# fudan-zvg/S-NeRF

Hardware: AMD Instinct MI355X
Metric: rays/sec (train step) (higher is better)
Workload: dtype bf16; 1 GPU; S-NeRF path A (MipNerfModel) train step, nuScenes-like 1600x900 rays, 64 proposal + 128 fine evals/ray (192 spp), hidden 1024, rgb_layer 3, cone + contraction + IPE-96

## Files before the change

include/snerf_hip.h:

```cpp
#ifndef SNERF_HIP_H
#define SNERF_HIP_H
#ifdef __cplusplus
extern "C" {
#endif

#define SNERF_DT_F32 0
#define SNERF_DT_BF16 1
#define SNERF_DT_F16 2
#define SNERF_DT_F64 3
#define SNERF_DT_BF16X3 4
#define SNERF_ACT_NONE 0
#define SNERF_ACT_RELU 1
#define SNERF_ACT_MASK 2
#define SNERF_ACT_RELU_BITS 3
#define SNERF_ACT_MASK_BITS 4

int snerf_version(void);
int snerf_last_hip_error(void);
int snerf_debug_lds_scribble(int seed, void* stream);

int snerf_linear_fwd(const void* A, long lda, const void* W, long ldw, const float* bias, void* Y, long ldy,
                     const void* aux, long ldaux, float* colsum, float* colsum_ws, int M, int N, int K, int n_store,
                     int act, int dtype, int out_f32, int variant, void* stream);

// ... 241 lines not shown
                             void* const* bits, void* const* dz, const long* dz_ld, float* const* g_bias, float* ws, long ws_floats, long M,
                             int dtype, void* stream);
int snerf_fcolour_fwd(const void* CB, long ldCB, const void* wstream, long n_frags, const float* bias, int n_blocks, float* raw_rgb,
                      void* const* acts, const long* act_ld, void* const* bits, long M, int variant, void* stream);
long snerf_fcolour_bwd_ws_floats(long M);
int snerf_fcolour_bwd(const float* d_raw_rgb, const void* wstream, long n_frags, void* const* bits, void* const* dC, const long* dC_ld,
                      void* dB, long dB_ld, float* const* g_bias, float* ws, long ws_floats, long M, void* stream);
int snerf_fcolour_fwd_dt(const void* CB, long ldCB, const void* wstream, long n_frags, const float* bias, int n_blocks, float* raw_rgb,
                         void* const* acts, const long* act_ld, void* const* bits, long M, int variant, int dtype, void* stream);
int snerf_fcolour_bwd_dt(const float* d_raw_rgb, const void* wstream, long n_frags, void* const* bits, void* const* dC, const long* dC_ld,
                         void* dB, long dB_ld, float* const* g_bias, float* ws, long ws_floats, long M, int dtype, void* stream);

long snerf_fchain_bwd_ws_floats(int net, long M);
int snerf_fchain_bwd(int net, const float* d_raw, const void* wstream, long n_frags, void* const* bits, void* const* dz, const long* dz_ld,
                     float* const* g_bias, float* ws, long ws_floats, long M, void* stream);
int snerf_fchain_bwd_dt(int net, const float* d_raw, const void* wstream, long n_frags, void* const* bits, void* const* dz, const long* dz_ld,
                        float* const* g_bias, float* ws, long ws_floats, long M, int dtype, void* stream);

long snerf_linear_wgrad_ws_floats(int M, int N, int K, long ldz, long ldx, int dtype, int variant);
int snerf_linear_wgrad_det(const void* Z, long ldz, const void* X, long ldx, float* dW, long ldw, const void* zeros, int M, int N, int K,
                           int n_valid, int k_valid, int dtype, int variant, float* ws, long ws_floats, void* stream);
int snerf_colsum_f32_det(const float* x, long ld, long M, int C, float* out, void* stream);

int snerf_classic_get_rays(int H, int W, double focal, double cx, double cy, const float* c2w_host, float* rays_o, float* rays_d, void* stream);
int snerf_classic_ndc_rays(int H, int W, double focal, float near, const float* rays_o, const float* rays_d, long n, float* o_out,
                           float* d_out, void* stream);
int snerf_classic_ray_batch(int H, int W, double focal, double cx, double cy, const float* c2w_host, const float* c2w_static_host,
                            const float* rays_o, const float* rays_d, long n, int ndc, float near, float far, const float* depths,
                            int use_viewdirs, float* rows, int ld, void* stream);

int snerf_zip_encode_bwd_binned(int pass, const float* tdist, const float* origins, const float* directions, const float* radii,
                                const float* base_x, const float* base_y, const float* deg_jitter, const int* offsets,
                                const int* grid_sizes, const void* grad_feat, long ld, float* grad_table, long R, int S, int L, int C, int n,
                                int m, float Sl, int H, float std_scale, int feat_dtype, const int* ksplit_host, const int* level_rows_host,
                                int* counts, void* wg_offsets, const long* starts, void* rec_row, float* rec_val, long capacity, void* g64,
                                long g64_rows, const int* scale_exp, void* stream);
int snerf_colsum_wide_f32(const float* x, long ld, long M, int C, float* out, int deterministic, void* stream);
int snerf_zip_glo_modulate(const void* X, long ldx, const float* SS, long ldss, long R, int S, int B, void* out, long ldo, int dtype, void* stream);
int snerf_zip_glo_modulate_bwd(const void* dXm, long lddxm, const void* X, long ldx, const float* SS, long ldss, const float* d_head, long ldh,
                               int n_head, long R, int S, int B, void* dX, long lddx, float* dSS, long lddss, float* dxsum, long ldsum,
                               int dtype, void* stream);
int snerf_zip_bin_scale(const void* grad_feat, long ld, long rows, int cols, int feat_dtype, int* scale_exp, void* stream);

int snerf_zip_encode_ray_bwd(const float* tdist, const float* origins, const float* directions, const float* radii, const float* base_x,
                             const float* base_y, const float* deg_jitter, const void* table, const int* offsets, const int* grid_sizes,
                             const void* grad_feat, long ld, long R, int S, int L, int C, int n, int m, float Sl, int H, float std_scale,
// ... 28 lines not shown
```

snerf_amd/csrc/elementwise.hip:

```cpp
#include "common.h"

struct AdamArgs {
  float lr, b1, b2, eps, grad_scale, grad_max_val;
  int zero_grad, nonfinite;
  const int* step_dev;
  const float* lr_dev;
  const float* clip_coef;
  int step;
  unsigned long long* dropped;
};

__device__ __forceinline__ float adam_clean_grad(float g, const AdamArgs& a, float coef) {
  g *= a.grad_scale * coef;
  if (a.grad_max_val > 0.f && g == g) g = fminf(fmaxf(g, -a.grad_max_val), a.grad_max_val);
  if (a.nonfinite == 1) g = (fabsf(g) <= 3.402823466e+38f) ? g : 0.f;
  else if (a.nonfinite == 2) g = (g != g) ? 0.f : fminf(fmaxf(g, -3.402823466e+38f), 3.402823466e+38f);
  return g;
}

__device__ __forceinline__ void adam_update(float& p, float& m, float& v, float gk, float b1, float b2, float step_size, float bc2_sqrt, float eps) {
#pragma clang fp contract(off)
  m = b1 * m + (1.f - b1) * gk;
  v = b2 * v + ((1.f - b2) * gk) * gk;
  p = p - (step_size * m) / (sqrtf(v) / bc2_sqrt + eps);
// ... 480 lines not shown
      (n_tiles > 0 && (tiles == nullptr || (((uintptr_t)tiles) & 15)))) return SNERF_ERR_ARG;
  if (n_b < 0 || (n_b > 0 && (idx_b == nullptr || dst_b == nullptr || (((uintptr_t)idx_b) & 15)))) return SNERF_ERR_ARG;
  const long want = (n + 1023) / 1024, want_b = (n_b + 1023) / 1024;
  const int gblocks = (int)(want < 4096 ? want : 4096), tblocks = (n_tiles + 3) / 4, bblocks = (int)(want_b < 1024 ? want_b : 1024);
  const dim3 g((unsigned)(gblocks + tblocks + bblocks)), b(256);
  const PackTile* tl = (const PackTile*)tiles;
  hipStream_t s = (hipStream_t)stream;
  if (dtype == SNERF_DT_F32) hipLaunchKernelGGL(gather_pack_tiles_kernel<float>, g, b, 0, s, flat, idx, n, (float*)dst, tl, n_tiles, tblocks, gblocks, idx_b, n_b, dst_b);
  else if (dtype == SNERF_DT_BF16) hipLaunchKernelGGL(gather_pack_tiles_kernel<__bf16>, g, b, 0, s, flat, idx, n, (__bf16*)dst, tl, n_tiles, tblocks, gblocks, idx_b, n_b, dst_b);
  else if (dtype == SNERF_DT_F16) hipLaunchKernelGGL(gather_pack_tiles_kernel<_Float16>, g, b, 0, s, flat, idx, n, (_Float16*)dst, tl, n_tiles, tblocks, gblocks, idx_b, n_b, dst_b);
  else return SNERF_ERR_ARG;
  return snerf_check_launch();
}

extern "C" int snerf_gather_pack_tiles(const float* flat, const int* idx, long n, void* dst, int dtype, const int* tiles, int n_tiles, void* stream) {
  return gather_pack_launch(flat, idx, n, dst, dtype, tiles, n_tiles, nullptr, 0, nullptr, stream);
}

extern "C" int snerf_gather_pack_pair(const float* flat, const int* idx, long n, void* dst, int dtype, const int* tiles, int n_tiles, const int* idx32,
                                      long n32, float* dst32, void* stream) {
  return gather_pack_launch(flat, idx, n, dst, dtype, tiles, n_tiles, idx32, n32, dst32, stream);
}

extern "C" int snerf_version() { return 3; }
int g_snerf_last_hip_error = 0;
extern "C" int snerf_last_hip_error() { return g_snerf_last_hip_error; }

__global__ __launch_bounds__(1024) void lds_scribble_kernel(unsigned seed, unsigned* sink) {
  extern __shared__ unsigned scribble[];
  unsigned h = seed * 2654435761u + blockIdx.x * 40503u + 17u;
  for (int i = threadIdx.x; i < 160 * 1024 / 4; i += 1024) {
    h = (h ^ (unsigned)i) * 1664525u + 1013904223u;
    scribble[i] = (h >> 7) ^ (h << 13);
  }
  __syncthreads();
  if (scribble[(seed + threadIdx.x) % (160 * 1024 / 4)] == 0x5eed5eedu && sink != nullptr) sink[0] = seed;
}
extern "C" int snerf_debug_lds_scribble(int seed, void* stream) {
  static bool attr = false;
  if (!attr) { (void)hipFuncSetAttribute((const void*)lds_scribble_kernel, hipFuncAttributeMaxDynamicSharedMemorySize, 160 * 1024); attr = true; }
  hipLaunchKernelGGL(lds_scribble_kernel, dim3(4096), dim3(1024), 160 * 1024, (hipStream_t)stream, (unsigned)seed, (unsigned*)nullptr);
  return snerf_check_launch();
}

__global__ __launch_bounds__(256) void split8_cast_kernel(const float* __restrict__ src, long ld_src, long M, int C, int G, _Float16* __restrict__ dst,
                                                          long ld_dst, int weight) {
  typedef _Float16 f16x8 __attribute__((ext_vector_type(8)));
// ... 34 lines not shown
```

snerf_amd/csrc/gemm.hip:

```cpp
#include "common.h"
#include <cstdlib>
#include <type_traits>

#define ACT_NONE 0
#define ACT_RELU 1
#define ACT_MASK 2
typedef unsigned short u16x2 __attribute__((ext_vector_type(2)));
#define ACT_RELU_BITS 3
#define ACT_MASK_BITS 4

typedef unsigned u32x4 __attribute__((ext_vector_type(4)));
typedef unsigned u32x2 __attribute__((ext_vector_type(2)));

struct GemmNT {
  const void* A; long lda;
  const void* W; long ldw;
  const float* bias;
  void* Y; long ldy;
  const void* aux; long ldaux;
  float* colsum;
  int M, N, K, n_store, act, out_f32, vec_store;
  float* colsum_ws; int fast_epi;
  int det;
  int dbg;
// ... 1223 lines not shown
    if ((variant & 1) && N % 256 == 0) return launch_nt<__bf16, 256, 256, 2, 4, true>(p, s);
    return launch_nt<__bf16, 128, 128, 2, 2, true>(p, s);
  }
  if (p8) return launch_nt8p(p, s);
  if (dtype == SNERF_DT_BF16 && (variant & 12) && N % 256 == 0) return launch_nt8(p, s);
  if (dtype == SNERF_DT_F32) return launch_nt<float, 128, 128, 2, 2>(p, s);
  if ((variant & 1) && N % 256 == 0) return launch_nt<__bf16, 256, 256, 2, 4>(p, s);
  return launch_nt<__bf16, 128, 128, 2, 2>(p, s);
}

struct GemmTN {
  const void* Z; long ldz;
  const void* X; long ldx;
  float* dW; long ldw;
  const void* zeros;
  int M, N, K, n_valid, k_valid, m_chunk;
  int tiles, slices;
  int split;
  float* part;
  long part_stride;
  int part_ld;
};

template <typename T, bool TR, int TN_STAGES, bool F16 = false>
__global__ __launch_bounds__(256) void gemm_tn_kernel(GemmTN p) {
  extern __shared__ __attribute__((aligned(16))) char smem[];
  constexpr int EPC = 16 / (int)sizeof(T);
  constexpr int ROWB = 128 * (int)sizeof(T);
  constexpr int MT = sizeof(T) == 4 ? 16 : 32;
  constexpr int TILEB = MT * ROWB;
  constexpr int RPI = 1024 / ROWB;
  constexpr int LI = MT / RPI / 4;
  const int tid = threadIdx.x, lane = tid & 63;
  const int wave = __builtin_amdgcn_readfirstlane(tid >> 6);
  const int wn = wave >> 1, wk = wave & 1;
  const int tiles_k = (p.K + 127) / 128;
  const int ntile = p.tiles;
  int slice, tile;
  {
    const int b = (int)blockIdx.x, xcd = b & 7, idx = b >> 3;
    const int full = p.slices >> 3;
    const int extra = p.slices & 7;
    const int mine = full + (xcd < extra ? 1 : 0);
    if (idx >= mine * ntile) return;
    slice = (idx / ntile) * 8 + xcd;
    tile = idx % ntile;
// ... 104 lines not shown
#pragma unroll
          for (int j = 0; j < 2; ++j) mma32t<F16>(acc[i][j], a[i].v, b[j].v);
      }
    }
  }
#pragma unroll
  for (int i = 0; i < 2; ++i)
#pragma unroll
    for (int j = 0; j < 2; ++j) {
      int k = k0 + wk * 64 + j * 32 + (lane & 31);
      if (p.split == 1) k = ((k >> 7) << 6) | (k & 63);
#pragma unroll
      for (int r = 0; r < 16; ++r) {
        int n = n0 + wn * 64 + i * 32 + (r & 3) + 8 * (r >> 2) + 4 * (lane >> 5);
        if (p.split == 1) n = ((n >> 7) << 6) | (n & 63);
        if (n < p.n_valid && k < p.k_valid) {
          if (p.part != nullptr) p.part[(long)slice * p.part_stride + (long)n * p.part_ld + k] = acc[i][j][r];
          else atomicAdd(p.dW + (long)n * p.ldw + k, acc[i][j][r]);
        }
      }
    }
}

template <bool SPLIT, bool F16 = false>
__global__ __launch_bounds__(512) void gemm_tn8_kernel(GemmTN p) {
  extern __shared__ __attribute__((aligned(16))) char smem[];
  typedef __bf16 T;
  typedef __attribute__((address_space(3))) bf16x4* lds_b4;
  constexpr int HALF = 64 * 256;
  const int tid = threadIdx.x, lane = tid & 63;
  const int wave = __builtin_amdgcn_readfirstlane(tid >> 6);
  const int wr = wave >> 2, wc = wave & 3;
  const int tiles_k = (p.K + 255) >> 8, tiles_n = (p.N + 255) >> 8;
  const int ntile = tiles_k * tiles_n;
  const int id = xcd_remap((int)blockIdx.x, (int)gridDim.x);
  const int tile = id % ntile, chunk = id / ntile;
  const int n0 = (tile / tiles_k) << 8, k0 = (tile % tiles_k) << 8;
  const int mbeg = chunk * p.m_chunk;
  const int rows = min(p.M, mbeg + p.m_chunk) - mbeg;
  const int KT = (rows + 63) >> 6;
  const T* __restrict__ Z = (const T*)p.Z + (long)mbeg * p.ldz + n0;
  const bool xhi = !SPLIT && p.split == 2;
  const T* __restrict__ X = (const T*)p.X + (long)mbeg * p.ldx + (xhi ? 2 * k0 : k0);
  const int xcols = xhi ? ((p.K - 1) >> 6) * 128 + ((p.K - 1) & 63) + 1 - 2 * k0 : p.K - k0;
  const int zbytes = (rows - 1) * (int)p.ldz * 2 + (p.N - n0) * 2, xbytes = (rows - 1) * (int)p.ldx * 2 + xcols * 2;
  const int zstep = 64 * (int)p.ldz * 2, xstep = 64 * (int)p.ldx * 2;

  const int lrow = lane >> 4, lch = lane & 15;
  const int lc = (lch ^ (4 * lrow)) * 8;
  constexpr int xhalf = SPLIT ? 128 : 64;
  const int zcol = ((lc >> 6) * 128 + (lc & 63)) * 2;
  const int xcol = SPLIT ? (((lc >> 6) * 128) + ((lc >> 5) & 1) * 32 + (lc & 31)) * 2 : ((lc >> 5) * (xhi ? 128 : 64) + (lc & 31)) * 2;
  int zrel[2], xrel[2];
#pragma unroll
  for (int i = 0; i < 2; ++i) {
    const int r = (wave * 2 + i) * 4 + lrow;
    zrel[i] = r * (int)p.ldz * 2 + zcol;
    xrel[i] = r * (int)p.ldx * 2 + xcol;
  }
  int s_kt = 0;
  auto stage = [&](int db, int which) __attribute__((always_inline)) {
    char* dst = smem + (db * 4 + which) * HALF + wave * 2048;
    if (which < 2) {
      const int off = s_kt * zstep;
      const int left = zbytes - off;
      const __amdgpu_buffer_rsrc_t r = __builtin_amdgcn_make_buffer_rsrc((void*)((const char*)Z + off), 0, left > 0 ? left : 0, 0x00020000);
      __builtin_amdgcn_raw_ptr_buffer_load_lds(r, (lds_ptr_t)dst, 16, zrel[0] + which * 128, 0, 0, 0);
      __builtin_amdgcn_raw_ptr_buffer_load_lds(r, (lds_ptr_t)(dst + 1024), 16, zrel[1] + which * 128, 0, 0, 0);
    } else {
      const int off = s_kt * xstep;
      const int left = xbytes - off;
      const __amdgpu_buffer_rsrc_t r = __builtin_amdgcn_make_buffer_rsrc((void*)((const char*)X + off), 0, left > 0 ? left : 0, 0x00020000);
      __builtin_amdgcn_raw_ptr_buffer_load_lds(r, (lds_ptr_t)dst, 16, xrel[0] + (which - 2) * xhalf, 0, 0, 0);
      __builtin_amdgcn_raw_ptr_buffer_load_lds(r, (lds_ptr_t)(dst + 1024), 16, xrel[1] + (which - 2) * xhalf, 0, 0, 0);
    }
  };

  const int g4 = lane >> 4, pl = lane & 15, prow = pl >> 2;
  const int frow = (8 * (g4 >> 1) + prow) * 256;
  const int fsub = ((pl & 1) << 3);
  int zc[2], xc1;
#pragma unroll
  for (int i2 = 0; i2 < 2; ++i2) zc[i2] = ((((wr * 64 + i2 * 32 + 16 * (g4 & 1)) >> 3) + ((pl & 3) >> 1)) ^ (4 * prow)) << 4;
  xc1 = ((((wc * 32 + 16 * (g4 & 1)) >> 3) + ((pl & 3) >> 1)) ^ (4 * prow)) << 4;
  bf16x8 aF[2][4], bS[2][4];
  const unsigned lds0 = (unsigned)(size_t)smem;
  auto lds_frag = [&](unsigned addr) __attribute__((always_inline)) {
    bf16x4 lo, hi;
    asm volatile("ds_read_b64_tr_b16 %0, %2\n\tds_read_b64_tr_b16 %1, %2 offset:1024" : "=&v"(lo), "=&v"(hi) : "v"(addr));
    return __builtin_shufflevector(lo, hi, 0, 1, 2, 3, 4, 5, 6, 7);
  };
  const unsigned za[2] = {lds0 + frow + zc[0] + fsub, lds0 + frow + zc[1] + fsub};
  const unsigned xa = lds0 + frow + xc1 + fsub;
  auto lds_a = [&](int db, int h, int i2, int ks) __attribute__((always_inline)) {
// ... 17 lines not shown
  };
  auto end_phase = [&]() __attribute__((always_inline)) {
    __builtin_amdgcn_sched_barrier(0);
    __builtin_amdgcn_s_barrier();
    __builtin_amdgcn_sched_barrier(0);
  };

  stage(0, 2); stage(0, 0); stage(0, 3); stage(0, 1);
  ++s_kt;
  stage(1, 3); stage(1, 0); stage(1, 2); stage(1, 1);
  ++s_kt;
  asm volatile("s_waitcnt vmcnt(10)" ::: "memory");
  __builtin_amdgcn_s_barrier();
#pragma unroll
  for (int ks = 0; ks < 4; ++ks) {
    aF[0][ks] = lds_a(0, 0, 0, ks);
    aF[1][ks] = lds_a(0, 0, 1, ks);
    bS[0][ks] = lds_b(0, 0, ks);
  }
  __builtin_amdgcn_s_waitcnt(0xC07F);
  __builtin_amdgcn_sched_barrier(0);
  __builtin_amdgcn_s_barrier();

  auto ktile = [&](auto db_tag) __attribute__((always_inline)) {
    constexpr int db = decltype(db_tag)::value;
    constexpr int F = db, S = 1 - db;
    if (wr == 1) { stage(db, 2 + F); wait_load(); }
#pragma unroll
    for (int ks = 0; ks < 4; ++ks) {
      bS[S][ks] = lds_b(db, S, ks);
      mma32t<F16>(acc[0][F], aF[0][ks], bS[F][ks]);
      mma32t<F16>(acc[1][F], aF[1][ks], bS[F][ks]);
      __builtin_amdgcn_sched_barrier(0);
    }
    if (wr == 0) { stage(db, 2 + F); wait_load(); }
    end_phase();
    if (wr == 1) { stage(db, 0); wait_load(); }
#pragma unroll
    for (int ks = 0; ks < 4; ++ks)
#pragma unroll
      for (int i2 = 0; i2 < 2; ++i2) {
        mma32t<F16>(acc[i2][S], aF[i2][ks], bS[S][ks]);
        aF[i2][ks] = lds_a(db, 1, i2, ks);
        __builtin_amdgcn_sched_barrier(0);
      }
    if (wr == 0) { stage(db, 0); wait_load(); }
    end_phase();
    if (wr == 1) { stage(db, 2 + S); wait_load(); }
    constexpr bool skip3 = S == 1 && SPLIT, skip4 = F == 1 && SPLIT;
#pragma unroll
    for (int ks = 0; ks < 4; ++ks) {
      if constexpr (!skip3) {
        mma32t<F16>(acc[2][S], aF[0][ks], bS[S][ks]);
        mma32t<F16>(acc[3][S], aF[1][ks], bS[S][ks]);
      }
      bS[S][ks] = lds_b(db ^ 1, S, ks);
      __builtin_amdgcn_sched_barrier(0);
    }
    if (wr == 0) { stage(db, 2 + S); wait_load(); }
    end_phase();
    if (wr == 1) { stage(db, 1); ++s_kt; wait_load(); }
#pragma unroll
    for (int ks = 0; ks < 4; ++ks)
#pragma unroll
      for (int i2 = 0; i2 < 2; ++i2) {
        if constexpr (!skip4) mma32t<F16>(acc[2 + i2][F], aF[i2][ks], bS[F][ks]);
        aF[i2][ks] = lds_a(db ^ 1, 0, i2, ks);
        __builtin_amdgcn_sched_barrier(0);
      }
    if (wr == 0) { stage(db, 1); ++s_kt; wait_load(); }
    end_phase();
  };
  for (int t = 0; t < KT; t += 2) {
    ktile(std::integral_constant<int, 0>{});
    if (t + 1 < KT) ktile(std::integral_constant<int, 1>{});
  }
  asm volatile("s_waitcnt vmcnt(0)" ::: "memory");

#pragma unroll
  for (int i = 0; i < 4; ++i)
#pragma unroll
    for (int j = 0; j < 2; ++j) {
      int k = k0 + wc * 64 + j * 32 + (lane & 31);
      if constexpr (SPLIT) {
        if (i >= 2 && j == 1) continue;
        k = k0 + (wc >> 1) * 128 + j * 64 + (wc & 1) * 32 + (lane & 31);
        k = ((k >> 7) << 6) | (k & 63);
      }
#pragma unroll
      for (int r = 0; r < 16; ++r) {
        int n = n0 + wr * 128 + i * 32 + (r & 3) + 8 * (r >> 2) + 4 * (lane >> 5);
        if constexpr (SPLIT) n = ((n >> 7) << 6) | (n & 63);
        if (n < p.n_valid && k < p.k_valid) {
          if (p.part != nullptr) p.part[(long)chunk * p.part_stride + (long)n * p.part_ld + k] = acc[i][j][r];
          else atomicAdd(p.dW + (long)n * p.ldw + k, acc[i][j][r]);
        }
      }
    }
}

// ... 40 lines not shown
#pragma unroll
  for (int w = 0; w < W; ++w) sm[g][lane][w] = s[w];
  __syncthreads();
  if (g == 0 && live) {
    float* dst = dW + (long)n * ldw + k;
#pragma unroll
    for (int w = 0; w < W; ++w) {
      float t = sm[0][lane][w];
#pragma unroll
      for (int q = 1; q < G; ++q) t += sm[q][lane][w];
      dst[w] += t;
    }
  }
}

struct TnPlan {
  bool use8;
  int slices;
  int m_chunk;
  int part_ld;
  long part_stride;
};

static TnPlan tn_plan(int M, int N, int K, long ldz, long ldx, int dtype, int variant, bool fold = false) {
  static int n_cu = 0;
  if (n_cu == 0) {
    int dev = 0;
    hipDeviceProp_t prop;
    n_cu = 256;
    if (hipGetDevice(&dev) == hipSuccess && hipGetDeviceProperties(&prop, dev) == hipSuccess && prop.multiProcessorCount > 0)
      n_cu = prop.multiProcessorCount;
  }
  TnPlan pl{};
  if ((variant & 2) && dtype == SNERF_DT_BF16 && N % 256 == 0 && K >= 256 && M >= 4096 && ldz * 2 * 65 < (1L << 31) && ldx * 2 * 65 < (1L << 31)) {
    const int t8 = (N / 256) * ((K + 255) / 256);
    int ch = n_cu / t8;
    ch = ch < 1 ? 1 : ch;
    long mc = ((long)M + ch - 1) / ch;
    mc = ((mc + 127) / 128) * 128;
    const long lim = (1L << 30) / ((ldz > ldx ? ldz : ldx) * 2);
    if (mc > lim) mc = lim / 128 * 128;
    if (!(fold && M <= 131072 && mc < 512)) {
      pl.use8 = true; pl.m_chunk = (int)mc; pl.slices = (int)((M + mc - 1) / mc);
      pl.part_ld = ((K + 255) / 256) * 256; pl.part_stride = (long)N * pl.part_ld;
      return pl;
    }
  }
  const int tiles = ((N + 127) / 128) * ((K + 127) / 128);
  const int target = (variant & 64) ? 4096 : (variant & 32) ? 2048 : (variant & 16) ? 512 : 1024;
  int chunks = (target + tiles - 1) / tiles;
  int m_chunk = (M + chunks - 1) / chunks;
  m_chunk = ((m_chunk + 255) / 256) * 256;
  const int floor_rows = (fold && M <= 131072) ? 256 : 1024;
  if (m_chunk < floor_rows) m_chunk = floor_rows;
  pl.use8 = false; pl.m_chunk = m_chunk; pl.slices = (M + m_chunk - 1) / m_chunk;
// ... 83 lines not shown
      hipLaunchKernelGGL(tn_fold_kernel<false>, dim3((k_valid + 255) / 256, n_valid), dim3(256), 0, (hipStream_t)stream, ws, pl.part_stride,
                         pl.part_ld, pl.slices, n_valid, k_valid, dW, ldw);
  }
  return snerf_check_launch();
}

extern "C" int snerf_linear_wgrad(const void* Z, long ldz, const void* X, long ldx, float* dW, long ldw, const void* zeros,
                                  int M, int N, int K, int n_valid, int k_valid, int dtype, int variant, void* stream) {
  return wgrad_launch(Z, ldz, X, ldx, dW, ldw, zeros, M, N, K, n_valid, k_valid, dtype, variant, nullptr, 0, stream);
}

extern "C" long snerf_linear_wgrad_ws_floats(int M, int N, int K, long ldz, long ldx, int dtype, int variant) {
  if (M <= 0 || N <= 0 || K <= 0) return 0;
  if (dtype == 2) dtype = SNERF_DT_BF16;
  const TnPlan pl = tn_plan(M, N, K, ldz, ldx, dtype, variant, true);
  return pl.part_stride * pl.slices;
}

extern "C" int snerf_linear_wgrad_det(const void* Z, long ldz, const void* X, long ldx, float* dW, long ldw, const void* zeros, int M, int N,
                                      int K, int n_valid, int k_valid, int dtype, int variant, float* ws, long ws_floats, void* stream) {
  if (ws == nullptr) return SNERF_ERR_ARG;
  return wgrad_launch(Z, ldz, X, ldx, dW, ldw, zeros, M, N, K, n_valid, k_valid, dtype, variant, ws, ws_floats, stream);
}
```

snerf_amd/mlp.py:

```python
import contextlib

import torch

from . import ops
from .ops import ACT_MASK, ACT_NONE, ACT_RELU, gran, roundup


class ParamArena:

    def __init__(self, shapes, device):
        self.names = [n for n, _ in shapes]
        self.shapes = dict(shapes)
        offs, o = {}, 0
        for n, s in shapes:
            numel = 1
            for d in s:
                numel *= d
            offs[n] = (o, numel)
            o += roundup(numel, 4)
        self.numel = roundup(o, 4)
        self._offs = offs
        self.epoch = 0
        self.flat = torch.zeros(self.numel, dtype=torch.float32, device=device)
        self.grad = torch.zeros(self.numel, dtype=torch.float32, device=device)
        self.p = {n: self.flat[a:a + c].view(self.shapes[n]) for n, (a, c) in offs.items()}
        self.g = {n: self.grad[a:a + c].view(self.shapes[n]) for n, (a, c) in offs.items()}

    def load(self, sd: dict, prefix: str = ""):
# ... 992 lines not shown
        else:
            cx, ck = CB, H + self.Cw
            for j in range(self.nc):
                cy = self.buf(M, self.cu)
                self.fwd(f"cond_layers.{j}.layers.0", cx, ck, cy, self.cu)
                cacts.append((cx, ck, cy))
                cx, ck = cy, self.cu
            self.fwd("rgb", cx, self.cu, raw_rgb, 3, ACT_NONE, out_f32=True)
        self.raw_sem, S0 = None, None
        if self.sc:
            S0 = self.buf(M, self.Hs)
            self.fwd("sem0", x, H, S0, self.Hs)
            self.raw_sem = self.buf(M, self.sc, f32=True)
            self.fwd("sem1", S0, self.Hs, self.raw_sem, self.sc, ACT_NONE, out_f32=True)
        return raw_rgb, raw_d, ((acts, cacts, SKIP, CB, S0) if keep else None)

    def backward(self, d_raw_rgb, d_raw_density, saved, d_raw_sem=None, want_input_grad=False, want_cond_grad=False, on_done=None):
        with self._bwd():
            if self._fp16_backward():
                return self._scaled_backward([d_raw_rgb, d_raw_density, d_raw_sem],
                                             lambda g: self._backward(g[0], g[1], saved, g[2], want_input_grad, want_cond_grad, None), on_done)
            return self._backward(d_raw_rgb, d_raw_density, saved, d_raw_sem, want_input_grad, want_cond_grad, on_done)

    def _backward(self, d_raw_rgb, d_raw_density, saved, d_raw_sem=None, want_input_grad=False, want_cond_grad=False, on_done=None):
        acts, cacts, SKIP, CB, S0 = saved
        H, g, cu, M = self.H, self.g, self.cu, d_raw_rgb.shape[0]
        dV = None
        DZE = self.buf(M, H * len(self.enc_layers)) if want_input_grad else None
        self.colsum(d_raw_rgb, 3, self.gB("rgb_layer"))
        self.colsum(d_raw_density, 1, self.gB("density_layer"))
        dz = self.head_grad(d_raw_rgb, 3)
        fused = cacts[-1] if (len(cacts) == self.nc + 1 and cacts[-1][0] == "fused") else None
        if fused is not None:
            cacts = cacts[:-1]
        clast = cacts[-1][2]
        self.wgrad("rgb_layer", dz, clast, 3, cu)
        DB = self.buf(M, H + g + (self.Hs if self.sc else 0))
        if fused is not None:
            _, cbits, bbits = fused
            dCs = [self.buf(M, cu) for _ in range(self.nc)]
            ops.fcolour_bwd(d_raw_rgb, self._cbwd[0], [cbits[2], cbits[1], cbits[0], bbits], dCs, self.cs(DB, 0, H),
                            [self.gB("cond_layers.2.layers.0"), self.gB("cond_layers.1.layers.0"), self.gB("cond_layers.0.layers.0"),
                             self.gB("bottleneck_layer.layers.0")])
            for j in range(self.nc - 1, -1, -1):
                cx, ck, cy = cacts[j]
                self.wgrad(f"cond_layers.{j}.layers.0", dCs[self.nc - 1 - j], cx, cu, H + self.cd if j == 0 else cu)
            if want_input_grad or want_cond_grad:
                dV = self.input_grad("cenc", dCs[-1], cu, self.Cw)
        else:
            dC = self.buf(M, cu)
            self.dgrad("rgb", dz, g, dC, cu, mask=clast, colsum=self.gB(f"cond_layers.{self.nc - 1}.layers.0"))
            for j in range(self.nc - 1, -1, -1):
                cx, ck, cy = cacts[j]
                n = f"cond_layers.{j}.layers.0"
                self.wgrad(n, dC, cx, cu, H + self.cd if j == 0 else cu)
                if j > 0:
                    dX = self.buf(M, cu)
                    self.dgrad(n, dC, cu, dX, cu, mask=cx, colsum=self.gB(f"cond_layers.{j - 1}.layers.0"))
                    dC = dX
                else:
                    self.dgrad(n, dC, cu, DB, H, mask=CB, colsum=self.gB("bottleneck_layer.layers.0"))
                    if want_input_grad or want_cond_grad:
                        dV = self.input_grad("cenc", dC, cu, self.Cw)
        ops.cast_pad(d_raw_density, 1, self.cs(DB, H, H + g), g, self.dt)
        xl = acts[-1][2]
        kb = H + g
        if self.sc:
            dS0 = self.cs(DB, H + g)
            if d_raw_sem is None:
                dS0.zero_()
            else:
                self.colsum(d_raw_sem, self.sc, self.gB("semantic_layer.1"))
                dzs = self.head_grad(d_raw_sem, self.sc)
                self.wgrad("semantic_layer.1", dzs, S0, self.sc, self.Hs)
                self.dgrad("sem1", dzs, roundup(self.sc, g), dS0, self.Hs, mask=S0, colsum=self.gB("semantic_layer.0.layers.0"))
                self.wgrad("semantic_layer.0.layers.0", dS0, xl, self.Hs, H)
            kb += self.Hs
        self.wgrad("bottleneck_layer.layers.0", self.cs(DB, 0, H), xl, H, H)
        self.wgrad("density_layer", self.cs(DB, H, H + g), xl, 1, H)
        dZ = self.buf(M, H)
        self.dgrad("bd", DB, kb, dZ, H, mask=xl, colsum=self.gB(f"layers.{self.L - 1}.layers.0"))
        if on_done is not None:
            on_done(["density_layer", "bottleneck_layer", "cond_layers", "rgb_layer"] + (["semantic_layer"] if self.sc else []))
        for i in range(self.L - 1, -1, -1):
            x, k, y = acts[i]
            n = f"layers.{i}.layers.0"
            self.wgrad(n, dZ, x, H, self.fd if i == 0 else (H + self.fd if self._is_skip_in(i) else H))
            if on_done is not None:
                on_done([f"layers.{i}."])
            if i > 0:
                xin = acts[i - 1][2]
                if want_input_grad and (i - 1) in self.enc_layers:
                    k = self.enc_layers.index(i - 1)
                    dX = self.cs(DZE, k * H, (k + 1) * H)
                else:
                    dX = self.buf(M, H)
                self.dgrad(n, dZ, H, dX, H, mask=xin, colsum=self.gB(f"layers.{i - 1}.layers.0"))
                dZ = dX
        if want_input_grad:
            return self.input_grad("enc", DZE, H * len(self.enc_layers), self.Ew), dV
        return dV if want_cond_grad else None


class ZipPropNet(_Net):

    def __init__(self, arena, prefix, dt, feat_dim, hidden=64, variant=8):
        super().__init__(arena, prefix, dt, variant)
        assert self.km == 1, "split-bf16 (compute='bf16x3') is built for the mip path's networks"
        assert hidden % self.g == 0
        import os
# ... 276 lines not shown
```

snerf_amd/ops.py:

```python
import ctypes
import os as _os

import torch

from . import _lib

F32, BF16, F16, F64 = 0, 1, 2, 3
BF16X3 = 4
F16F8 = 5
SPLIT_DTS = (BF16X3, F16F8)
ACT_NONE, ACT_RELU, ACT_MASK = 0, 1, 2
ACT_RELU_BITS, ACT_MASK_BITS = 3, 4
_TORCH_DT = {F32: torch.float32, BF16: torch.bfloat16, F16: torch.float16, BF16X3: torch.bfloat16, F16F8: torch.float16}


def torch_dtype(dt: int):
    return _TORCH_DT[dt]


def gran(dt: int) -> int:
    return 32 if dt == F32 else 64


def roundup(x: int, m: int) -> int:
# ... 98 lines not shown


def linear_wgrad(dZ, X, dW, n_valid, k_valid, dt, variant=0, deterministic=False, x_split_hi=False):
    _chk2d(dZ, _TORCH_DT[dt]); _chk2d(X, _TORCH_DT[dt]); _chk2d(dW, torch.float32)
    assert dZ.shape[0] == X.shape[0] and dW.shape[0] >= n_valid and dW.shape[1] >= k_valid
    Kx = X.shape[1]
    if x_split_hi:
        assert dt in (BF16, F16) and Kx % 128 == 0
        Kx //= 2
        variant |= 1 << 14
    if dt == BF16X3:
        assert not deterministic, "the split-bf16 weight gradient has no deterministic fold"
        assert dZ.shape[1] % 128 == 0 and X.shape[1] % 128 == 0
    if not deterministic and wgrad_uses_fold(dZ.shape[0], dZ.shape[1], Kx, dt, variant, n_valid, k_valid):
        deterministic = True
    if deterministic:
        nws = _lib.query("snerf_linear_wgrad_ws_floats", dZ.shape[0], dZ.shape[1], Kx, dZ.stride(0), X.stride(0), dt, variant)
        ws = torch.empty(max(int(nws), 1), dtype=torch.float32, device=dZ.device)
        _lib.call("snerf_linear_wgrad_det", _p(dZ), dZ.stride(0), _p(X), X.stride(0), _p(dW), dW.stride(0), _p(zero_page(dZ.device)),
                  dZ.shape[0], dZ.shape[1], Kx, n_valid, k_valid, dt, variant, _p(ws), ws.numel(), _stream())
        return
    _lib.call("snerf_linear_wgrad", _p(dZ), dZ.stride(0), _p(X), X.stride(0), _p(dW), dW.stride(0),
              _p(zero_page(dZ.device)), dZ.shape[0], dZ.shape[1], Kx, n_valid, k_valid, dt, variant, _stream())


def _fmlp_dt(stream):
    assert stream.dtype in (torch.bfloat16, torch.float16) and stream.is_contiguous(), "the fused 256-wide networks run in bf16 or fp16"
    return stream.dtype, _zip_dt(stream)


def fmlp_classic_fwd(E, VE, stream, bias, raw):
    tdt, dt = _fmlp_dt(stream)
    _chk2d(E, tdt); _chk2d(VE, tdt); _chk2d(raw, torch.float32)
    assert bias.dtype == torch.float32 and raw.is_contiguous() and raw.shape[1] == 4
    assert E.shape[1] >= 64 and VE.shape[1] >= 32 and VE.shape[0] == E.shape[0] == raw.shape[0]
    _lib.call("snerf_fmlp_classic_fwd_dt", _p(E), E.stride(0), _p(VE), VE.stride(0), _p(stream), stream.shape[0], _p(bias), bias.numel() // 32,
              _p(raw), E.shape[0], dt, _stream())


def fmlp_classic_pts_fwd(pts, viewdirs, S, stream, bias, raw):
    _f32c(pts); _chk2d(raw, torch.float32)
    _, dt = _fmlp_dt(stream)
    assert viewdirs.dtype == torch.float32 and viewdirs.stride(1) == 1 and viewdirs.shape[1] == 3 and pts.shape[0] == viewdirs.shape[0] * S
    assert bias.dtype == torch.float32 and raw.is_contiguous() and raw.shape == (pts.shape[0], 4)
    _lib.call("snerf_fmlp_classic_pts_fwd_dt", _p(pts), _p(viewdirs), viewdirs.stride(0), int(S), _p(stream), stream.shape[0], _p(bias),
              bias.numel() // 32, _p(raw), pts.shape[0], dt, _stream())
# ... 1243 lines not shown
```

Measured before the change: 162,900 rays/s.

## Add edge-tile weight-gradient GEMM with half-tile edges and merged bottleneck/density wgrad

Adds an edge-aware variant of the 256x256 TN weight-gradient kernel. Tiles whose valid N or K extent is at most 128 get half-width processing that skips MMAs and loads, and the M-split is weighted per tile class to balance work across CUs, followed by a separate fold kernel. In the MLP backward, it is used for the first trunk layer, the first cond layer, and a single merged launch covering both the bottleneck and density weight gradients, cutting wasted padded-tile work and launch count. In exchange it adds a workspace allocation per call, an extra fold pass, and more complex indexing logic.

```diff
diff --git a/include/snerf_hip.h b/include/snerf_hip.h
--- a/include/snerf_hip.h
+++ b/include/snerf_hip.h
@@ -287,6 +287,11 @@
                            int n_valid, int k_valid, int dtype, int variant, float* ws, long ws_floats, void* stream);
 int snerf_colsum_f32_det(const float* x, long ld, long M, int C, float* out, void* stream);
 
+long snerf_linear_wgrad_edge_ws_floats(int M, int N, int K, int n_valid, int k_valid, long ldz, long ldx, int dtype, int variant);
+int snerf_linear_wgrad_edge_plan(int M, int N, int K, int n_valid, int k_valid, long ldz, long ldx, int dtype, int variant, int* out);
+int snerf_linear_wgrad_edge(const void* Z, long ldz, const void* X, long ldx, float* dW, long ldw, float* dW2, long ldw2, int n_split,
+                            int M, int N, int K, int n_valid, int k_valid, int dtype, int variant, float* ws, long ws_floats, void* stream);
+
 int snerf_classic_get_rays(int H, int W, double focal, double cx, double cy, const float* c2w_host, float* rays_o, float* rays_d, void* stream);
 int snerf_classic_ndc_rays(int H, int W, double focal, float near, const float* rays_o, const float* rays_d, long n, float* o_out,
                            float* d_out, void* stream);
diff --git a/snerf_amd/csrc/elementwise.hip b/snerf_amd/csrc/elementwise.hip
--- a/snerf_amd/csrc/elementwise.hip
+++ b/snerf_amd/csrc/elementwise.hip
@@ -526,7 +526,7 @@
   return gather_pack_launch(flat, idx, n, dst, dtype, tiles, n_tiles, idx32, n32, dst32, stream);
 }
 
-extern "C" int snerf_version() { return 3; }
+extern "C" int snerf_version() { return 4; }
 int g_snerf_last_hip_error = 0;
 extern "C" int snerf_last_hip_error() { return g_snerf_last_hip_error; }
 
diff --git a/snerf_amd/csrc/gemm.hip b/snerf_amd/csrc/gemm.hip
--- a/snerf_amd/csrc/gemm.hip
+++ b/snerf_amd/csrc/gemm.hip
@@ -1269,6 +1269,15 @@
   int part_ld;
 };
 
+struct GemmTNE : GemmTN {
+  int tk, tn;
+  int kedge, nedge;
+  int ctiles[4];
+  int cslices[4];
+  int cchunk[4];
+  long cbase[4];
+};
+
 template <typename T, bool TR, int TN_STAGES, bool F16 = false>
 __global__ __launch_bounds__(256) void gemm_tn_kernel(GemmTN p) {
   extern __shared__ __attribute__((aligned(16))) char smem[];
@@ -1419,8 +1428,9 @@
     }
 }
 
-template <bool SPLIT, bool F16 = false>
-__global__ __launch_bounds__(512) void gemm_tn8_kernel(GemmTN p) {
+template <bool SPLIT, bool F16 = false, bool EDGE = false>
+__global__ __launch_bounds__(512) void gemm_tn8_kernel(std::conditional_t<EDGE, GemmTNE, GemmTN> p) {
+  static_assert(!(EDGE && SPLIT), "edge tiles: plain 16-bit operands");
   extern __shared__ __attribute__((aligned(16))) char smem[];
   typedef __bf16 T;
   typedef __attribute__((address_space(3))) bf16x4* lds_b4;
@@ -1431,10 +1441,27 @@
   const int tiles_k = (p.K + 255) >> 8, tiles_n = (p.N + 255) >> 8;
   const int ntile = tiles_k * tiles_n;
   const int id = xcd_remap((int)blockIdx.x, (int)gridDim.x);
-  const int tile = id % ntile, chunk = id / ntile;
-  const int n0 = (tile / tiles_k) << 8, k0 = (tile % tiles_k) << 8;
-  const int mbeg = chunk * p.m_chunk;
-  const int rows = min(p.M, mbeg + p.m_chunk) - mbeg;
+  int tile = id % ntile, chunk = id / ntile;
+  int n0 = (tile / tiles_k) << 8, k0 = (tile % tiles_k) << 8;
+  int m_chunk = p.m_chunk;
+  int cls = 0, cnt = 0;
+  if constexpr (EDGE) {
+    int cid = id;
+#pragma unroll
+    for (int c = 0; c < 3; ++c) {
+      const int wgs = p.ctiles[c] * p.cslices[c];
+      if (cls == c && cid >= wgs) { cid -= wgs; cls = c + 1; }
+    }
+    cnt = cls == 0 ? p.ctiles[0] : cls == 1 ? p.ctiles[1] : cls == 2 ? p.ctiles[2] : p.ctiles[3];
+    m_chunk = cls == 0 ? p.cchunk[0] : cls == 1 ? p.cchunk[1] : cls == 2 ? p.cchunk[2] : p.cchunk[3];
+    tile = cid % cnt; chunk = cid / cnt;
+    const int fk = p.tk - p.kedge;
+    n0 = ((cls & 2) ? p.tn - 1 : ((cls & 1) ? tile : tile / fk)) << 8;
+    k0 = ((cls & 1) ? p.tk - 1 : ((cls & 2) ? tile : tile % fk)) << 8;
+  }
+  const bool ke = EDGE && (cls & 1), ne = EDGE && (cls & 2);
+  const int mbeg = chunk * m_chunk;
+  const int rows = min(p.M, mbeg + m_chunk) - mbeg;
   const int KT = (rows + 63) >> 6;
   const T* __restrict__ Z = (const T*)p.Z + (long)mbeg * p.ldz + n0;
   const bool xhi = !SPLIT && p.split == 2;
@@ -1446,8 +1473,8 @@
   const int lrow = lane >> 4, lch = lane & 15;
   const int lc = (lch ^ (4 * lrow)) * 8;
   constexpr int xhalf = SPLIT ? 128 : 64;
-  const int zcol = ((lc >> 6) * 128 + (lc & 63)) * 2;
-  const int xcol = SPLIT ? (((lc >> 6) * 128) + ((lc >> 5) & 1) * 32 + (lc & 31)) * 2 : ((lc >> 5) * (xhi ? 128 : 64) + (lc & 31)) * 2;
+  const int zcol = ne ? lc * 2 : ((lc >> 6) * 128 + (lc & 63)) * 2;
+  const int xcol = ke ? lc * 2 : SPLIT ? (((lc >> 6) * 128) + ((lc >> 5) & 1) * 32 + (lc & 31)) * 2 : ((lc >> 5) * (xhi ? 128 : 64) + (lc & 31)) * 2;
   int zrel[2], xrel[2];
 #pragma unroll
   for (int i = 0; i < 2; ++i) {
@@ -1460,13 +1487,15 @@
     char* dst = smem + (db * 4 + which) * HALF + wave * 2048;
     if (which < 2) {
       const int off = s_kt * zstep;
-      const int left = zbytes - off;
+      int left = zbytes - off;
+      if constexpr (EDGE) { if (which == 1 && ne) left = 0; }
       const __amdgpu_buffer_rsrc_t r = __builtin_amdgcn_make_buffer_rsrc((void*)((const char*)Z + off), 0, left > 0 ? left : 0, 0x00020000);
       __builtin_amdgcn_raw_ptr_buffer_load_lds(r, (lds_ptr_t)dst, 16, zrel[0] + which * 128, 0, 0, 0);
       __builtin_amdgcn_raw_ptr_buffer_load_lds(r, (lds_ptr_t)(dst + 1024), 16, zrel[1] + which * 128, 0, 0, 0);
     } else {
       const int off = s_kt * xstep;
-      const int left = xbytes - off;
+      int left = xbytes - off;
+      if constexpr (EDGE) { if (which == 3 && ke) left = 0; }
       const __amdgpu_buffer_rsrc_t r = __builtin_amdgcn_make_buffer_rsrc((void*)((const char*)X + off), 0, left > 0 ? left : 0, 0x00020000);
       __builtin_amdgcn_raw_ptr_buffer_load_lds(r, (lds_ptr_t)dst, 16, xrel[0] + (which - 2) * xhalf, 0, 0, 0);
       __builtin_amdgcn_raw_ptr_buffer_load_lds(r, (lds_ptr_t)(dst + 1024), 16, xrel[1] + (which - 2) * xhalf, 0, 0, 0);
@@ -1530,15 +1559,19 @@
   __builtin_amdgcn_sched_barrier(0);
   __builtin_amdgcn_s_barrier();
 
-  auto ktile = [&](auto db_tag) __attribute__((always_inline)) {
+  auto ktile = [&](auto db_tag, auto cls_tag) __attribute__((always_inline)) {
     constexpr int db = decltype(db_tag)::value;
     constexpr int F = db, S = 1 - db;
+    constexpr bool KE = (decltype(cls_tag)::value & 1) != 0, NE = (decltype(cls_tag)::value & 2) != 0;
+    constexpr bool xF = !(KE && F == 1), xS = !(KE && S == 1);
     if (wr == 1) { stage(db, 2 + F); wait_load(); }
 #pragma unroll
     for (int ks = 0; ks < 4; ++ks) {
       bS[S][ks] = lds_b(db, S, ks);
-      mma32t<F16>(acc[0][F], aF[0][ks], bS[F][ks]);
-      mma32t<F16>(acc[1][F], aF[1][ks], bS[F][ks]);
+      if constexpr (xF) {
+        mma32t<F16>(acc[0][F], aF[0][ks], bS[F][ks]);
+        mma32t<F16>(acc[1][F], aF[1][ks], bS[F][ks]);
+      }
       __builtin_amdgcn_sched_barrier(0);
     }
     if (wr == 0) { stage(db, 2 + F); wait_load(); }
@@ -1548,14 +1581,14 @@
     for (int ks = 0; ks < 4; ++ks)
 #pragma unroll
       for (int i2 = 0; i2 < 2; ++i2) {
-        mma32t<F16>(acc[i2][S], aF[i2][ks], bS[S][ks]);
+        if constexpr (xS) mma32t<F16>(acc[i2][S], aF[i2][ks], bS[S][ks]);
         aF[i2][ks] = lds_a(db, 1, i2, ks);
         __builtin_amdgcn_sched_barrier(0);
       }
     if (wr == 0) { stage(db, 0); wait_load(); }
     end_phase();
     if (wr == 1) { stage(db, 2 + S); wait_load(); }
-    constexpr bool skip3 = S == 1 && SPLIT, skip4 = F == 1 && SPLIT;
+    constexpr bool skip3 = (S == 1 && SPLIT) || NE || !xS, skip4 = (F == 1 && SPLIT) || NE || !xF;
 #pragma unroll
     for (int ks = 0; ks < 4; ++ks) {
       if constexpr (!skip3) {
@@ -1579,11 +1612,43 @@
     if (wr == 0) { stage(db, 1); ++s_kt; wait_load(); }
     end_phase();
   };
-  for (int t = 0; t < KT; t += 2) {
-    ktile(std::integral_constant<int, 0>{});
-    if (t + 1 < KT) ktile(std::integral_constant<int, 1>{});
+  auto run = [&](auto cls_tag) __attribute__((always_inline)) {
+    for (int t = 0; t < KT; t += 2) {
+      ktile(std::integral_constant<int, 0>{}, cls_tag);
+      if (t + 1 < KT) ktile(std::integral_constant<int, 1>{}, cls_tag);
+    }
+  };
+  if constexpr (!EDGE) {
+    for (int t = 0; t < KT; t += 2) {
+      ktile(std::integral_constant<int, 0>{}, std::integral_constant<int, 0>{});
+      if (t + 1 < KT) ktile(std::integral_constant<int, 1>{}, std::integral_constant<int, 0>{});
+    }
+  } else {
+    if (cls == 0) run(std::integral_constant<int, 0>{});
+    else if (cls == 1) run(std::integral_constant<int, 1>{});
+    else if (cls == 2) run(std::integral_constant<int, 2>{});
+    else run(std::integral_constant<int, 3>{});
   }
   asm volatile("s_waitcnt vmcnt(0)" ::: "memory");
+
+  if constexpr (EDGE) {
+    const int pld = ke ? 128 : 256;
+    const long base = cls == 0 ? p.cbase[0] : cls == 1 ? p.cbase[1] : cls == 2 ? p.cbase[2] : p.cbase[3];
+    float* part = p.part + base + ((long)chunk * cnt + tile) * ((ne ? 128 : 256) * pld);
+#pragma unroll
+    for (int i = 0; i < 4; ++i)
+#pragma unroll
+      for (int j = 0; j < 2; ++j) {
+        if ((ne && i >= 2) || (ke && j == 1)) continue;
+        const int kl = (ke ? wc * 32 : wc * 64 + j * 32) + (lane & 31);
+#pragma unroll
+        for (int r = 0; r < 16; ++r) {
+          const int nl = (ne ? wr * 64 + (i & 1) * 32 : wr * 128 + i * 32) + (r & 3) + 8 * (r >> 2) + 4 * (lane >> 5);
+          if (n0 + nl < p.n_valid && k0 + kl < p.k_valid) part[nl * pld + kl] = acc[i][j][r];
+        }
+      }
+    return;
+  }
 
 #pragma unroll
   for (int i = 0; i < 4; ++i)
@@ -1670,7 +1735,7 @@
   long part_stride;
 };
 
-static TnPlan tn_plan(int M, int N, int K, long ldz, long ldx, int dtype, int variant, bool fold = false) {
+static int tn_cu_count() {
   static int n_cu = 0;
   if (n_cu == 0) {
     int dev = 0;
@@ -1679,6 +1744,11 @@
     if (hipGetDevice(&dev) == hipSuccess && hipGetDeviceProperties(&prop, dev) == hipSuccess && prop.multiProcessorCount > 0)
       n_cu = prop.multiProcessorCount;
   }
+  return n_cu;
+}
+
+static TnPlan tn_plan(int M, int N, int K, long ldz, long ldx, int dtype, int variant, bool fold = false) {
+  const int n_cu = tn_cu_count();
   TnPlan pl{};
   if ((variant & 2) && dtype == SNERF_DT_BF16 && N % 256 == 0 && K >= 256 && M >= 4096 && ldz * 2 * 65 < (1L << 31) && ldx * 2 * 65 < (1L << 31)) {
     const int t8 = (N / 256) * ((K + 255) / 256);
@@ -1808,3 +1878,154 @@
   if (ws == nullptr) return SNERF_ERR_ARG;
   return wgrad_launch(Z, ldz, X, ldx, dW, ldw, zeros, M, N, K, n_valid, k_valid, dtype, variant, ws, ws_floats, stream);
 }
+
+struct TnFoldE {
+  const float* part;
+  int tk, tn, kedge, nedge;
+  int ctiles[4], cslices[4];
+  long cbase[4];
+  int n_valid, k_valid, n_split;
+  float* dW; long ldw;
+  float* dW2; long ldw2;
+};
+
+template <bool VEC>
+__global__ __launch_bounds__(256) void tn_fold_edge_kernel(TnFoldE p) {
+  const int k = (blockIdx.x * 256 + threadIdx.x) * (VEC ? 4 : 1), n = blockIdx.y;
+  if (k >= p.k_valid || n >= p.n_valid) return;
+  const int tr = n >> 8, tc = k >> 8;
+  const bool ne = p.nedge && tr == p.tn - 1, ke = p.kedge && tc == p.tk - 1;
+  const int cls = (ne ? 2 : 0) | (ke ? 1 : 0);
+  const int tile = ne ? (ke ? 0 : tc) : (ke ? tr : tr * (p.tk - p.kedge) + tc);
+  const int cnt = cls == 0 ? p.ctiles[0] : cls == 1 ? p.ctiles[1] : cls == 2 ? p.ctiles[2] : p.ctiles[3];
+  const int slices = cls == 0 ? p.cslices[0] : cls == 1 ? p.cslices[1] : cls == 2 ? p.cslices[2] : p.cslices[3];
+  const long base = cls == 0 ? p.cbase[0] : cls == 1 ? p.cbase[1] : cls == 2 ? p.cbase[2] : p.cbase[3];
+  const int pld = ke ? 128 : 256;
+  const long image = (long)(ne ? 128 : 256) * pld, stride = image * cnt;
+  const float* src = p.part + base + tile * image + (n & 255) * pld + (k & 255);
+  float* dst = n < p.n_split ? p.dW + (long)n * p.ldw + k : p.dW2 + (long)(n - p.n_split) * p.ldw2 + k;
+  if constexpr (VEC) {
+    f32x4 s = {0.f, 0.f, 0.f, 0.f};
+#pragma unroll 8
+    for (int c = 0; c < slices; ++c) s += *(const f32x4*)(src + c * stride);
+    *(f32x4*)dst += s;
+  } else {
+    float s = 0.f;
+    for (int c = 0; c < slices; ++c) s += src[c * stride];
+    *dst += s;
+  }
+}
+
+struct TnEdgePlan {
+  int N, K;
+  int tk, tn, kedge, nedge;
+  int ctiles[4], cslices[4], cchunk[4];
+  long cbase[4];
+  long ws_floats;
+  int wgs;
+};
+
+static const int TN_EDGE_WEIGHT = 6;
+
+static bool tn_edge_plan(int M, int N, int K, int n_valid, int k_valid, long ldz, long ldx, int dtype, int variant, TnEdgePlan& pl) {
+  pl = TnEdgePlan{};
+  if (dtype != SNERF_DT_BF16 && dtype != 2) return false;
+  if (M < 4096 || N < 8 || K < 8 || N % 8 || K % 8 || ldz % 8 || ldx % 8 || ldz < N || ldx < K) return false;
+  if (!(N >= 256 || K >= 256 || (N >= 128 && K >= 128))) return false;
+  if (n_valid < 1 || n_valid > N || k_valid < 1 || k_valid > K) return false;
+  if (ldz * 2 * 65 >= (1L << 31) || ldx * 2 * 65 >= (1L << 31)) return false;
+  pl.N = (n_valid + 7) / 8 * 8; pl.K = (k_valid + 7) / 8 * 8;
+  pl.tn = (pl.N + 255) / 256; pl.tk = (pl.K + 255) / 256;
+  const bool probe_full = (variant & 1) != 0;
+  pl.nedge = !probe_full && n_valid - (pl.tn - 1) * 256 <= 128;
+  pl.kedge = !probe_full && k_valid - (pl.tk - 1) * 256 <= 128;
+  const int fn = pl.tn - pl.nedge, fk = pl.tk - pl.kedge;
+  pl.ctiles[0] = fn * fk; pl.ctiles[1] = pl.kedge ? fn : 0; pl.ctiles[2] = pl.nedge ? fk : 0; pl.ctiles[3] = pl.nedge && pl.kedge;
+  const int n_cu = tn_cu_count();
+  const int cap = (M + 127) / 128;
+  const int we = ((variant >> 1) & 15) ? ((variant >> 1) & 15) : TN_EDGE_WEIGHT;
+  const int TN_EDGE_WEIGHT[4] = {8, we, we, (we * we + 4) / 8};
+  int units = 0, total = 0;
+  for (int c = 0; c < 4; ++c) units += TN_EDGE_WEIGHT[c] * pl.ctiles[c];
+  int S[4];
+  for (int c = 0; c < 4; ++c) {
+    S[c] = 0;
+    if (!pl.ctiles[c]) continue;
+    S[c] = n_cu * TN_EDGE_WEIGHT[c] / units;
+    S[c] = S[c] < 1 ? 1 : (S[c] > cap ? cap : S[c]);
+    total += S[c] * pl.ctiles[c];
+  }
+  for (;;) {
+    int pick = -1;
+    long worst = 0;
+    for (int c = 0; c < 4; ++c) {
+      if (!pl.ctiles[c] || S[c] >= cap || total + pl.ctiles[c] > n_cu) continue;
+      const long cost = (long)TN_EDGE_WEIGHT[c] * ((M + S[c] - 1) / S[c]);
+      if (cost > worst) { worst = cost; pick = c; }
+    }
+    if (pick < 0) break;
+    ++S[pick]; total += pl.ctiles[pick];
+  }
+  const long lim = (1L << 30) / ((ldz > ldx ? ldz : ldx) * 2);
+  long at = 0;
+  for (int c = 0; c < 4; ++c) {
+    if (!pl.ctiles[c]) continue;
+    long mc = ((long)M + S[c] - 1) / S[c];
+    mc = (mc + 127) / 128 * 128;
+    if (mc > lim) mc = lim / 128 * 128;
+    pl.cchunk[c] = (int)mc; pl.cslices[c] = (int)((M + mc - 1) / mc);
+    pl.cbase[c] = at;
+    at += (long)pl.cslices[c] * pl.ctiles[c] * ((c & 2) ? 128 : 256) * ((c & 1) ? 128 : 256);
+    pl.wgs += pl.cslices[c] * pl.ctiles[c];
+  }
+  pl.ws_floats = at;
+  return true;
+}
+
+extern "C" long snerf_linear_wgrad_edge_ws_floats(int M, int N, int K, int n_valid, int k_valid, long ldz, long ldx, int dtype, int variant) {
+  TnEdgePlan pl;
+  return tn_edge_plan(M, N, K, n_valid, k_valid, ldz, ldx, dtype, variant, pl) ? pl.ws_floats : 0;
+}
+
+extern "C" int snerf_linear_wgrad_edge_plan(int M, int N, int K, int n_valid, int k_valid, long ldz, long ldx, int dtype, int variant, int* out) {
+  TnEdgePlan pl;
+  if (out == nullptr || !tn_edge_plan(M, N, K, n_valid, k_valid, ldz, ldx, dtype, variant, pl)) return SNERF_ERR_ARG;
+  for (int c = 0; c < 4; ++c) { out[c] = pl.ctiles[c]; out[4 + c] = pl.cslices[c]; out[8 + c] = pl.cchunk[c]; }
+  out[12] = pl.tk; out[13] = pl.tn; out[14] = pl.wgs;
+  return SNERF_OK;
+}
+
+extern "C" int snerf_linear_wgrad_edge(const void* Z, long ldz, const void* X, long ldx, float* dW, long ldw, float* dW2, long ldw2, int n_split,
+                                       int M, int N, int K, int n_valid, int k_valid, int dtype, int variant, float* ws, long ws_floats,
+                                       void* stream) {
+  TnEdgePlan pl;
+  if (Z == nullptr || X == nullptr || dW == nullptr || ws == nullptr || ((size_t)Z & 15) || ((size_t)X & 15)) return SNERF_ERR_ARG;
+  if (!tn_edge_plan(M, N, K, n_valid, k_valid, ldz, ldx, dtype, variant, pl) || ws_floats < pl.ws_floats) return SNERF_ERR_ARG;
+  if (dW2 == nullptr) n_split = n_valid;
+  else if (n_split < 1 || n_split >= n_valid) return SNERF_ERR_ARG;
+  GemmTNE p{};
+  p.Z = Z; p.ldz = ldz; p.X = X; p.ldx = ldx; p.dW = dW; p.ldw = ldw;
+  p.M = M; p.N = pl.N; p.K = pl.K; p.n_valid = n_valid; p.k_valid = k_valid;
+  p.part = ws;
+  p.tk = pl.tk; p.tn = pl.tn; p.kedge = pl.kedge; p.nedge = pl.nedge;
+  TnFoldE f{};
+  f.part = ws; f.tk = pl.tk; f.tn = pl.tn; f.kedge = pl.kedge; f.nedge = pl.nedge;
+  for (int c = 0; c < 4; ++c) {
+    p.ctiles[c] = f.ctiles[c] = pl.ctiles[c]; p.cslices[c] = f.cslices[c] = pl.cslices[c]; p.cchunk[c] = pl.cchunk[c];
+    p.cbase[c] = f.cbase[c] = pl.cbase[c];
+  }
+  f.n_valid = n_valid; f.k_valid = k_valid; f.n_split = n_split; f.dW = dW; f.ldw = ldw; f.dW2 = dW2; f.ldw2 = ldw2;
+  static bool attr_set = false;
+  if (!attr_set) {
+    hipFuncSetAttribute((const void*)gemm_tn8_kernel<false, false, true>, hipFuncAttributeMaxDynamicSharedMemorySize, 8 * 64 * 256);
+    hipFuncSetAttribute((const void*)gemm_tn8_kernel<false, true, true>, hipFuncAttributeMaxDynamicSharedMemorySize, 8 * 64 * 256);
+    attr_set = true;
+  }
+  if (dtype == 2) hipLaunchKernelGGL((gemm_tn8_kernel<false, true, true>), dim3(pl.wgs), dim3(512), 8 * 64 * 256, (hipStream_t)stream, p);
+  else hipLaunchKernelGGL((gemm_tn8_kernel<false, false, true>), dim3(pl.wgs), dim3(512), 8 * 64 * 256, (hipStream_t)stream, p);
+  const bool vec = k_valid % 4 == 0 && ldw % 4 == 0 && ((size_t)dW & 15) == 0 && ((size_t)ws & 15) == 0 &&
+                   (dW2 == nullptr || (ldw2 % 4 == 0 && ((size_t)dW2 & 15) == 0));
+  if (vec) hipLaunchKernelGGL(tn_fold_edge_kernel<true>, dim3((k_valid / 4 + 255) / 256, n_valid), dim3(256), 0, (hipStream_t)stream, f);
+  else hipLaunchKernelGGL(tn_fold_edge_kernel<false>, dim3((k_valid + 255) / 256, n_valid), dim3(256), 0, (hipStream_t)stream, f);
+  return snerf_check_launch();
+}
diff --git a/snerf_amd/mlp.py b/snerf_amd/mlp.py
--- a/snerf_amd/mlp.py
+++ b/snerf_amd/mlp.py
@@ -4,6 +4,9 @@
 
 from . import ops
 from .ops import ACT_MASK, ACT_NONE, ACT_RELU, gran, roundup
+
+WGRAD_EDGE_DEFAULT = "bd,c0,l0"
+WGRAD_EDGE = frozenset(r for r in __import__("os").environ.get("SNERF_WGRAD_EDGE", WGRAD_EDGE_DEFAULT).split(",") if r not in ("", "0"))
 
 
 class ParamArena:
@@ -1042,6 +1045,19 @@
                                              lambda g: self._backward(g[0], g[1], saved, g[2], want_input_grad, want_cond_grad, None), on_done)
             return self._backward(d_raw_rgb, d_raw_density, saved, d_raw_sem, want_input_grad, want_cond_grad, on_done)
 
+    WGRAD_EDGE_MIN_ROWS = 131072
+
+    def _wgrad_edge_ok(self, M):
+        return (not self._in_plain_bwd and self.dt in (ops.BF16, ops.F16) and not self.sc and M > self.WGRAD_EDGE_MIN_ROWS
+                and M >= 4096 and self.H >= 256)
+
+    def _wgrad_cond(self, j, dC, cx, M):
+        n, k = f"cond_layers.{j}.layers.0", (self.H + self.cd if j == 0 else self.cu)
+        if j == 0 and "c0" in WGRAD_EDGE and self._wgrad_edge_ok(M) and self.cu % 8 == 0 and self.cu <= 128:
+            ops.linear_wgrad_edge(dC, cx, self.gW(n), self.cu, k, self.dt)
+        else:
+            self.wgrad(n, dC, cx, self.cu, k)
+
     def _backward(self, d_raw_rgb, d_raw_density, saved, d_raw_sem=None, want_input_grad=False, want_cond_grad=False, on_done=None):
         acts, cacts, SKIP, CB, S0 = saved
         H, g, cu, M = self.H, self.g, self.cu, d_raw_rgb.shape[0]
@@ -1064,7 +1080,7 @@
                              self.gB("bottleneck_layer.layers.0")])
             for j in range(self.nc - 1, -1, -1):
                 cx, ck, cy = cacts[j]
-                self.wgrad(f"cond_layers.{j}.layers.0", dCs[self.nc - 1 - j], cx, cu, H + self.cd if j == 0 else cu)
+                self._wgrad_cond(j, dCs[self.nc - 1 - j], cx, M)
             if want_input_grad or want_cond_grad:
                 dV = self.input_grad("cenc", dCs[-1], cu, self.Cw)
         else:
@@ -1073,7 +1089,7 @@
             for j in range(self.nc - 1, -1, -1):
                 cx, ck, cy = cacts[j]
                 n = f"cond_layers.{j}.layers.0"
-                self.wgrad(n, dC, cx, cu, H + self.cd if j == 0 else cu)
+                self._wgrad_cond(j, dC, cx, M)
                 if j > 0:
                     dX = self.buf(M, cu)
                     self.dgrad(n, dC, cu, dX, cu, mask=cx, colsum=self.gB(f"cond_layers.{j - 1}.layers.0"))
@@ -1096,8 +1112,13 @@
                 self.dgrad("sem1", dzs, roundup(self.sc, g), dS0, self.Hs, mask=S0, colsum=self.gB("semantic_layer.0.layers.0"))
                 self.wgrad("semantic_layer.0.layers.0", dS0, xl, self.Hs, H)
             kb += self.Hs
-        self.wgrad("bottleneck_layer.layers.0", self.cs(DB, 0, H), xl, H, H)
-        self.wgrad("density_layer", self.cs(DB, H, H + g), xl, 1, H)
+        edge = WGRAD_EDGE if self._wgrad_edge_ok(M) else frozenset()
+        if "bd" in edge:
+            ops.linear_wgrad_edge(self.cs(DB, 0, H + g), xl, self.gW("bottleneck_layer.layers.0"), H + 1, H, self.dt,
+                                  dW2=self.gW("density_layer"), n_split=H)
+        else:
+            self.wgrad("bottleneck_layer.layers.0", self.cs(DB, 0, H), xl, H, H)
+            self.wgrad("density_layer", self.cs(DB, H, H + g), xl, 1, H)
         dZ = self.buf(M, H)
         self.dgrad("bd", DB, kb, dZ, H, mask=xl, colsum=self.gB(f"layers.{self.L - 1}.layers.0"))
         if on_done is not None:
@@ -1105,7 +1126,10 @@
         for i in range(self.L - 1, -1, -1):
             x, k, y = acts[i]
             n = f"layers.{i}.layers.0"
-            self.wgrad(n, dZ, x, H, self.fd if i == 0 else (H + self.fd if self._is_skip_in(i) else H))
+            if "l0" in edge and i == 0 and self.fd % 8 == 0:
+                ops.linear_wgrad_edge(dZ, x, self.gW(n), H, self.fd, self.dt)
+            else:
+                self.wgrad(n, dZ, x, H, self.fd if i == 0 else (H + self.fd if self._is_skip_in(i) else H))
             if on_done is not None:
                 on_done([f"layers.{i}."])
             if i > 0:
diff --git a/snerf_amd/ops.py b/snerf_amd/ops.py
--- a/snerf_amd/ops.py
+++ b/snerf_amd/ops.py
@@ -144,6 +144,29 @@
         return
     _lib.call("snerf_linear_wgrad", _p(dZ), dZ.stride(0), _p(X), X.stride(0), _p(dW), dW.stride(0),
               _p(zero_page(dZ.device)), dZ.shape[0], dZ.shape[1], Kx, n_valid, k_valid, dt, variant, _stream())
+
+
+def linear_wgrad_edge_plan(M, N, K, n_valid, k_valid, ldz, ldx, dt, variant=0):
+    out = (ctypes.c_int * 16)()
+    _lib.call("snerf_linear_wgrad_edge_plan", M, N, K, n_valid, k_valid, ldz, ldx, dt, variant, ctypes.cast(out, ctypes.c_void_p))
+    ws = _lib.query("snerf_linear_wgrad_edge_ws_floats", M, N, K, n_valid, k_valid, ldz, ldx, dt, variant)
+    return {"tiles": list(out[0:4]), "slices": list(out[4:8]), "rows": list(out[8:12]), "tiles_k": out[12], "tiles_n": out[13],
+            "workgroups": out[14], "ws_floats": int(ws)}
+
+
+def linear_wgrad_edge(dZ, X, dW, n_valid, k_valid, dt, dW2=None, n_split=0, variant=0):
+    _chk2d(dZ, _TORCH_DT[dt]); _chk2d(X, _TORCH_DT[dt]); _chk2d(dW, torch.float32)
+    assert dt in (BF16, F16) and dZ.shape[0] == X.shape[0] and dZ.shape[1] >= n_valid and X.shape[1] >= k_valid and dW.shape[1] >= k_valid
+    if dW2 is None:
+        assert dW.shape[0] >= n_valid
+    else:
+        _chk2d(dW2, torch.float32)
+        assert 0 < n_split < n_valid and dW.shape[0] >= n_split and dW2.shape[0] >= n_valid - n_split and dW2.shape[1] >= k_valid
+    M, N, K = dZ.shape[0], dZ.shape[1], X.shape[1]
+    nws = _lib.query("snerf_linear_wgrad_edge_ws_floats", M, N, K, n_valid, k_valid, dZ.stride(0), X.stride(0), dt, variant)
+    ws = torch.empty(max(int(nws), 4), dtype=torch.float32, device=dZ.device)
+    _lib.call("snerf_linear_wgrad_edge", _p(dZ), dZ.stride(0), _p(X), X.stride(0), _p(dW), dW.stride(0), _p(dW2),
+              0 if dW2 is None else dW2.stride(0), n_split, M, N, K, n_valid, k_valid, dt, variant, _p(ws), ws.numel(), _stream())
 
 
 def _fmlp_dt(stream):
```

Result: no change. 164,100 rays/s (median of 6 runs) (+0.7%).
